# phd3/presto-1

Measured on AMD Instinct MI355X. Metric: probe_rows_per_sec, higher is better.
Workload: dtype int64+f64

## Files before the change

### presto-1_amd/csrc/agg.hip

```cpp
#include "agg.h"
#include "kernels.h"
#include "device_agg.h"

#include <rocprim/rocprim.hpp>

#include <algorithm>
#include <cstdlib>

namespace tgpu {

namespace {

constexpr int kBlock = 256;

struct AggView {
    int32_t function;
    int32_t pad;
    const void *input;
    const uint8_t *input_nulls;
    const uint8_t *mask;
    const uint8_t *mask_nulls;
    const void *input2;
    const uint8_t *input2_nulls;
    long long *counts;
// ... 29 lines not shown
                if (cnt == 0) continue;
                atomicAdd((unsigned long long *)&a.counts[g], (unsigned long long)cnt);
                if (a.function == TGPU_AGG_SUM_BIGINT) i128_add(&a.i128[g * 2], ((const long long *)a.input2)[r]);
                else if (tg_is_minmax(a.function)) tg_minmax_update(&a.i128[g * 2], tg_minmax_encode(a.function, ((const unsigned long long *)a.input2)[r]));
                else kulisch_add(&a.limbs[g * kLimbs], &a.special[g], ((const double *)a.input2)[r]);
                continue;
            }
            if (a.mask && ((a.mask_nulls && a.mask_nulls[r]) || !a.mask[r])) continue;
            if (a.function == TGPU_AGG_COUNT_ALL) {
                atomicAdd((unsigned long long *)&a.counts[g], 1ULL);
                continue;
            }
            if (a.input_nulls && a.input_nulls[r]) continue;
            atomicAdd((unsigned long long *)&a.counts[g], 1ULL);
            switch (a.function) {
            case TGPU_AGG_SUM_BIGINT: i128_add(&a.i128[g * 2], ((const long long *)a.input)[r]); break;
            case TGPU_AGG_MIN_BIGINT:
            case TGPU_AGG_MAX_BIGINT:
            case TGPU_AGG_MIN_DOUBLE:
            case TGPU_AGG_MAX_DOUBLE: tg_minmax_update(&a.i128[g * 2], tg_minmax_encode(a.function, ((const unsigned long long *)a.input)[r])); break;
            case TGPU_AGG_SUM_DOUBLE:
            case TGPU_AGG_AVG_DOUBLE: kulisch_add(&a.limbs[g * kLimbs], &a.special[g], ((const double *)a.input)[r]); break;
            case TGPU_AGG_AVG_BIGINT: kulisch_add(&a.limbs[g * kLimbs], &a.special[g], (double)((const long long *)a.input)[r]); break;
            default: break;
            }
        }
    }
}


__global__ void __launch_bounds__(kBlock) ordered_keys_kernel(const int32_t *__restrict__ gids, int64_t n, unsigned int *__restrict__ keys, int *__restrict__ rows,
                                                               unsigned int *__restrict__ unsorted)
{
    bool bad = false;
    for (int64_t r = (int64_t)blockIdx.x * kBlock + threadIdx.x; r < n; r += (int64_t)gridDim.x * kBlock) {
        const int32_t g = gids[r];
        keys[r] = (unsigned int)(g + 1);
        rows[r] = (int)r;
        bad = bad || (r > 0 && gids[r - 1] > g);
    }
    if (unsorted && __any(bad) && (threadIdx.x & 63) == 0) *unsorted = 1u;
}

__global__ void __launch_bounds__(kBlock) ordered_stretches_kernel(const unsigned int *__restrict__ keys, int64_t n, int *__restrict__ stretches)
{
    for (int64_t i = (int64_t)blockIdx.x * kBlock + threadIdx.x; i < n; i += (int64_t)gridDim.x * kBlock) {
        const unsigned int k = keys[i];
        if (k == 0) continue;
        if (i == 0 || keys[i - 1] != k) stretches[(size_t)(k - 1) * 2] = (int)i;
        if (i == n - 1 || keys[i + 1] != k) stretches[(size_t)(k - 1) * 2 + 1] = (int)(i + 1);
    }
}

template <bool INTERMEDIATE>
__global__ void __launch_bounds__(kBlock) agg_ordered_kernel(AggArgs args, const unsigned int *__restrict__ keys, const int *__restrict__ rows, int64_t n,
                                                              unsigned int *error, int64_t handoff, long long *list, unsigned int *list_count)
{
    for (int64_t i = (int64_t)blockIdx.x * kBlock + threadIdx.x; i < n; i += (int64_t)gridDim.x * kBlock) {
        const unsigned int key = keys[i];
        if (key == 0 || (i > 0 && keys[i - 1] == key)) continue;
        const int64_t g = (int64_t)key - 1;
        const int64_t stop = handoff > 0 ? (i + handoff < n ? i + handoff : n) : n;
        if (handoff > 0 && stop < n && keys[stop] == key) {
            const unsigned int at = atomicAdd(list_count, 1u);
            list[(size_t)at * 2] = g;
            list[(size_t)at * 2 + 1] = stop;
        }
#pragma unroll
        for (int k = 0; k < kMaxAggs; k++) {
            if (k >= args.n_aggs) break;
            const AggView &a = args.a[k];
            long long cnt = 0;
            double s = a.dsum ? a.dsum[g] : 0.0;
            __int128 big = 0;
            unsigned long long best = 0;
            for (int64_t j = i; j < stop && keys[j] == key; j++) {
                const int64_t r = rows[j];
                if (INTERMEDIATE) {
                    const long long c = ((const long long *)a.input)[r];
                    if (c == 0) continue;
                    cnt += c;
                    if (a.function == TGPU_AGG_SUM_BIGINT) big += ((const long long *)a.input2)[r];
                    else if (tg_is_minmax(a.function)) {
                        const unsigned long long c_ = tg_minmax_encode(a.function, ((const unsigned long long *)a.input2)[r]);
                        best = c_ > best ? c_ : best;
                    }
                    else if (a.function != TGPU_AGG_COUNT_ALL && a.function != TGPU_AGG_COUNT_COLUMN) s += ((const double *)a.input2)[r];
                    continue;
                }
                if (a.mask && ((a.mask_nulls && a.mask_nulls[r]) || !a.mask[r])) continue;
                if (a.function != TGPU_AGG_COUNT_ALL && a.input_nulls && a.input_nulls[r]) continue;
                cnt++;
                switch (a.function) {
                case TGPU_AGG_SUM_BIGINT: big += ((const long long *)a.input)[r]; break;
                case TGPU_AGG_MIN_BIGINT:
                case TGPU_AGG_MAX_BIGINT:
                case TGPU_AGG_MIN_DOUBLE:
                case TGPU_AGG_MAX_DOUBLE: {
                    const unsigned long long c_ = tg_minmax_encode(a.function, ((const unsigned long long *)a.input)[r]);
                    best = c_ > best ? c_ : best;
                    break;
                }
                case TGPU_AGG_SUM_DOUBLE:
                case TGPU_AGG_AVG_DOUBLE: s += ((const double *)a.input)[r]; break;
                case TGPU_AGG_AVG_BIGINT: s += (double)((const long long *)a.input)[r]; break;
                default: break;
                }
            }
            if (cnt) a.counts[g] += cnt;
            if (a.dsum) a.dsum[g] = s;
            if (best) tg_minmax_update(&a.i128[g * 2], best);
            if (a.i128 && big != 0) {
                const unsigned __int128 cur = ((unsigned __int128)a.i128[g * 2 + 1] << 64) | a.i128[g * 2];
                const unsigned __int128 nxt = cur + (unsigned __int128)big;
                a.i128[g * 2] = (unsigned long long)nxt;
                a.i128[g * 2 + 1] = (unsigned long long)(nxt >> 64);
            }
        }
    }
    (void)error;
}

struct OrdChainPlan {
    int32_t slot[kMaxAggs];
};

__device__ inline long long wave_sum_i64(long long v)
{
#pragma unroll
    for (int d = 32; d >= 1; d >>= 1) v += __shfl_xor(v, d, 64);
    return v;
}

__device__ inline void ordered_chain_group(const AggArgs &args, const OrdChainPlan &plan, const int *__restrict__ rows, int64_t g, long long s, long long e, double *vals,
                                           unsigned long long *cnt_lds, unsigned long long *lo_lds, long long *hi_lds)
{
    const int wave = threadIdx.x >> 6, lane = threadIdx.x & 63;
    if (threadIdx.x < kMaxAggs) {
        cnt_lds[threadIdx.x] = 0;
        lo_lds[threadIdx.x] = 0;
        hi_lds[threadIdx.x] = 0;
    }
    double *sum = nullptr;
    if (wave == 0) {
        __builtin_amdgcn_s_setprio(3);
#pragma unroll
        for (int k = 0; k < kMaxAggs; k++)
            if (k < args.n_aggs && plan.slot[k] == lane) sum = args.a[k].dsum;
    }
    double os = sum ? sum[g] : 0.0;
    __syncthreads();
    const long long tiles = (e - s + TG_ORD_TILE - 1) / TG_ORD_TILE;
    const int r = (wave - 1) * 64 + lane;
    long long row_next = (wave > 0 && s + r < e) ? rows[s + r] : 0;
    for (long long t = 0; t <= tiles; t++) {
        if (wave > 0 && t < tiles) {
            const long long j = s + t * TG_ORD_TILE + r;
            const long long row = row_next;
            if (j + TG_ORD_TILE < e) row_next = rows[j + TG_ORD_TILE];
            double *out = vals + (t & 1) * (TG_ORD_MAX_DOUBLES * TG_ORD_STRIDE) + r;
            const bool live = j < e;
#pragma unroll
            for (int k = 0; k < kMaxAggs; k++) {
                if (k >= args.n_aggs) break;
                const AggView &a = args.a[k];
                bool take = live;
                if (take && a.mask && ((a.mask_nulls && a.mask_nulls[row]) || !a.mask[row])) take = false;
                if (take && a.function != TGPU_AGG_COUNT_ALL && a.input_nulls && a.input_nulls[row]) take = false;
                const unsigned long long taken = __ballot(take);
                if (lane == 0 && taken) atomicAdd(&cnt_lds[k], (unsigned long long)__popcll(taken));
                if (a.function == TGPU_AGG_SUM_BIGINT) {
                    const long long v = take ? ((const long long *)a.input)[row] : 0;
                    const long long lo = wave_sum_i64((long long)(unsigned int)v), hi = wave_sum_i64(v >> 32);
                    if (lane == 0 && taken) {
                        atomicAdd(&lo_lds[k], (unsigned long long)lo);
                        atomicAdd((unsigned long long *)&hi_lds[k], (unsigned long long)hi);
                    }
                }
                else if (tg_is_minmax(a.function)) {
                    if (take) tg_minmax_update(&a.i128[g * 2], tg_minmax_encode(a.function, ((const unsigned long long *)a.input)[row]));
                }
                else if (plan.slot[k] >= 0 && live) {
                    double x = -0.0;
                    if (take) x = a.function == TGPU_AGG_AVG_BIGINT ? (double)((const long long *)a.input)[row] : ((const double *)a.input)[row];
                    out[plan.slot[k] * TG_ORD_STRIDE] = x;
                }
            }
        }
        else if (wave == 0 && t > 0 && sum) {
            const long long left = e - (s + (t - 1) * TG_ORD_TILE);
            os = tg_chain_add_tile(vals + ((t - 1) & 1) * (TG_ORD_MAX_DOUBLES * TG_ORD_STRIDE) + lane * TG_ORD_STRIDE, left < TG_ORD_TILE ? (int)left : TG_ORD_TILE, os);
        }
        __syncthreads();
    }
    if (sum) sum[g] = os;
    if (threadIdx.x == 64) {
#pragma unroll
        for (int k = 0; k < kMaxAggs; k++) {
            if (k >= args.n_aggs) break;
            const AggView &a = args.a[k];
            if (cnt_lds[k]) a.counts[g] += (long long)cnt_lds[k];
            if (a.function == TGPU_AGG_SUM_BIGINT && a.i128) {
                const __int128 big = (__int128)hi_lds[k] * ((__int128)1 << 32) + (__int128)lo_lds[k];
                const unsigned __int128 cur = ((unsigned __int128)a.i128[g * 2 + 1] << 64) | a.i128[g * 2];
                const unsigned __int128 nxt = cur + (unsigned __int128)big;
                a.i128[g * 2] = (unsigned long long)nxt;
                a.i128[g * 2 + 1] = (unsigned long long)(nxt >> 64);
            }
        }
    }
    __syncthreads();
}

__global__ void __launch_bounds__(TG_ORD_WAVES * 64) agg_ordered_chain_kernel(AggArgs args, OrdChainPlan plan, const int *__restrict__ stretches,
                                                                               const unsigned int *__restrict__ keys, const int *__restrict__ rows, int64_t n,
                                                                               const long long *__restrict__ list, const unsigned int *__restrict__ list_count)
{
    __shared__ __attribute__((aligned(16))) double vals[2 * TG_ORD_MAX_DOUBLES * TG_ORD_STRIDE];
    __shared__ unsigned long long cnt_lds[kMaxAggs], lo_lds[kMaxAggs];
    __shared__ long long hi_lds[kMaxAggs];
    if (stretches) {
        const long long s = stretches[(size_t)blockIdx.x * 2], e = stretches[(size_t)blockIdx.x * 2 + 1];
        if (e > s) ordered_chain_group(args, plan, rows, blockIdx.x, s, e, vals, cnt_lds, lo_lds, hi_lds);
        return;
    }
    const unsigned int count = *list_count;
    for (unsigned int b = blockIdx.x; b < count; b += gridDim.x) {
        const long long g = list[(size_t)b * 2], s = list[(size_t)b * 2 + 1];
        long long lo = s, hi = n;
        while (lo < hi) { const long long mid = (lo + hi) >> 1; if (keys[mid] <= (unsigned int)(g + 1)) lo = mid + 1; else hi = mid; }
        if (lo > s) ordered_chain_group(args, plan, rows, g, s, lo, vals, cnt_lds, lo_lds, hi_lds);
    }
}

using LowCardPlan = TgLowCardPlan;

struct LowCardStates {
    TgAggState st[kMaxAggs];
};

__global__ void __launch_bounds__(kBlock) agg_lowcard_kernel(AggArgs args, LowCardStates states, LowCardPlan plan, const int32_t *__restrict__ gids, int64_t n,
                                                              TgFoldScratch fold)
{
    extern __shared__ __attribute__((aligned(16))) unsigned char lds[];
    tg_lc_zero(lds, plan);
    for (int64_t r = (int64_t)blockIdx.x * kBlock + threadIdx.x; r < n; r += (int64_t)gridDim.x * kBlock) {
        const int g = gids ? gids[r] : 0;
        if (g < 0) continue;
        double *hi_base = tg_lc_hi(lds, plan, g), *lo_base = tg_lc_lo(lds, plan, g);
        unsigned int *cnt_base = tg_lc_cnt(lds, plan, g);
        for (int k = 0; k < args.n_aggs; k++) {
            const AggView &a = args.a[k];
            if (a.mask && ((a.mask_nulls && a.mask_nulls[r]) || !a.mask[r])) continue;
            if (a.function != TGPU_AGG_COUNT_ALL && a.input_nulls && a.input_nulls[r]) continue;
            cnt_base[plan.cnt_slot[k] * kBlock + threadIdx.x] += 1u;
            if (tg_is_minmax(a.function)) {
                tg_minmax_update(&a.i128[(size_t)g * 2], tg_minmax_encode(a.function, ((const unsigned long long *)a.input)[r]));
                continue;
            }
            const int w = plan.wide_slot[k];
            if (w < 0) continue;
            if (a.function == TGPU_AGG_SUM_BIGINT) {
                tg_lc_add_bigint(hi_base, lo_base, w, ((const long long *)a.input)[r]);
                continue;
            }
            const double v = a.function == TGPU_AGG_AVG_BIGINT ? (double)((const long long *)a.input)[r] : ((const double *)a.input)[r];
            if (!(fabs(v) <= 1.7976931348623157e308)) {
                tg_flag_special(&a.special[g], v);
                continue;
            }
            const double r = tg_lc_add_double(hi_base, lo_base, w, v);
            if (r != 0.0) tg_kulisch_add(&a.limbs[(size_t)g * kLimbs], &a.special[g], r);
        }
    }
    tg_lc_fold(lds, plan, states.st, fold);
}

__global__ void __launch_bounds__(kBlock) agg_fold_flush_kernel(TgFoldScratch fs, int rows, int n_aggs, LowCardStates states)
{
    tg_fold_flush(fs, rows, n_aggs, states.st);
}

struct KulischWindow {
    int top;
// ... 517 lines not shown
    HIP_CHECK(rocprim::radix_sort_pairs(temp->ptr(), temp_bytes, keys_in->as<unsigned int>(), keys->as<unsigned int>(), rows_in->as<int>(), rows->as<int>(), (size_t)n, 0,
                                        end_bit, ctx_->stream()));
}

void GroupedAccumulators::add_input(const int32_t *gids, int64_t n, const DevicePage &page, int64_t group_count, bool gids_ascending)
{
    if (states_.empty() || n <= 0) return;
    BufferPtr zero_gids;
    if (!gids && force_ordered()) {
        zero_gids = ctx_->alloc_zero((size_t)n * 4);
        gids = zero_gids->as<int32_t>();
    }
    if (gids) decide_mode(group_count > 0 ? group_count : 1, (160 * 1024) / std::max<int64_t>(lowcard_bytes_per_group(specs()), 1));
    else if (mode_ == Mode::UNDECIDED) mode_ = Mode::EXACT;
    {
        const int64_t lowcard_capacity = (160 * 1024) / std::max<int64_t>(lowcard_bytes_per_group(specs()), 1);
        const int64_t g = group_count > 0 ? group_count : 1;
        ensure(mode_ == Mode::EXACT && g <= lowcard_capacity ? lowcard_capacity : g);
    }
    AggArgs args{};
    args.n_aggs = (int32_t)states_.size();
    for (size_t k = 0; k < states_.size(); k++) {
        State &st = states_[k];
        AggView &a = args.a[k];
        a.function = st.spec.function;
        if (st.spec.function != TGPU_AGG_COUNT_ALL) {
            int32_t want = 0;
            if (bigint_valued(st.spec.function) || st.spec.function == TGPU_AGG_AVG_BIGINT) want = TGPU_BIGINT;
            if (st.spec.function == TGPU_AGG_MIN_DOUBLE || st.spec.function == TGPU_AGG_MAX_DOUBLE) want = TGPU_DOUBLE;
            if (st.spec.function == TGPU_AGG_SUM_DOUBLE || st.spec.function == TGPU_AGG_AVG_DOUBLE) want = TGPU_DOUBLE;
            check_channel(page, st.spec.input_channel, want, "aggregate input");
            a.input = page.cols[st.spec.input_channel].values;
            a.input_nulls = page.cols[st.spec.input_channel].nulls;
        }
        if (st.spec.mask_channel >= 0) {
            check_channel(page, st.spec.mask_channel, TGPU_BOOLEAN, "aggregate mask");
            a.mask = (const uint8_t *)page.cols[st.spec.mask_channel].values;
            a.mask_nulls = page.cols[st.spec.mask_channel].nulls;
        }
        a.counts = st.counts->as<long long>();
        a.limbs = st.limbs ? st.limbs->as<long long>() : nullptr;
        a.special = st.special ? st.special->as<unsigned int>() : nullptr;
        a.i128 = st.i128 ? st.i128->as<unsigned long long>() : nullptr;
        a.dsum = st.dsum ? st.dsum->as<double>() : nullptr;
    }
    if (mode_ == Mode::ORDERED) {
        TG_CHECK_STATE(gids != nullptr, "ordered accumulation needs group ids");
        OrdChainPlan plan{};
        int doubles = 0;
        for (int k = 0; k < kMaxAggs; k++) plan.slot[k] = (k < args.n_aggs && args.a[k].dsum) ? doubles++ : -1;
        const int64_t ids = group_count > 0 ? group_count : 1;
        const bool chained = doubles <= TG_ORD_MAX_DOUBLES && ids <= ord_chain_max_groups() && n >= ids * kOrdChainMinRows && getenv("TGPU_DISABLE_ORDERED_CHAIN") == nullptr;
        ProfileScope ps(ctx_, chained ? "agg_accumulate_ordered_chain" : "agg_accumulate_ordered");
        BufferPtr keys, rows;
        sort_rows_by_group(gids, n, group_count, keys, rows, gids_ascending);
        if (chained) {
            BufferPtr stretches = group_stretches(keys->as<unsigned int>(), n, ids);
            agg_ordered_chain_kernel<<<(int)ids, TG_ORD_WAVES * 64, 0, ctx_->stream()>>>(args, plan, stretches->as<int>(), keys->as<unsigned int>(), rows->as<int>(), n, nullptr,
                                                                                          nullptr);
            check_launch("agg_accumulate_ordered_chain");
            return;
        }
        const int64_t long_groups = n / kOrdHandoffRows;
        const bool handoff = long_groups > 0 && doubles <= TG_ORD_MAX_DOUBLES && getenv("TGPU_DISABLE_ORDERED_CHAIN") == nullptr;
        BufferPtr list = handoff ? ctx_->alloc((size_t)long_groups * 16) : nullptr, list_count = handoff ? ctx_->alloc_zero(8) : nullptr;
        agg_ordered_kernel<false><<<grid_for(ctx_, n), kBlock, 0, ctx_->stream()>>>(args, keys->as<unsigned int>(), rows->as<int>(), n, error_->as<unsigned int>(),
                                                                                      handoff ? kOrdHandoffRows : 0, handoff ? list->as<long long>() : nullptr,
                                                                                      handoff ? list_count->as<unsigned int>() : nullptr);
        check_launch("agg_accumulate_ordered");
        if (handoff) {
            agg_ordered_chain_kernel<<<(int)std::min<int64_t>(long_groups, ctx_->cu_count()), TG_ORD_WAVES * 64, 0, ctx_->stream()>>>(
                args, plan, nullptr, keys->as<unsigned int>(), rows->as<int>(), n, list->as<long long>(), list_count->as<unsigned int>());
            check_launch("agg_accumulate_ordered_handoff");
        }
        return;
    }
    LowCardPlan plan{};
    plan.n_aggs = args.n_aggs;
    for (int k = 0; k < args.n_aggs; k++) {
        plan.wide_slot[k] = (is_count(args.a[k].function) || is_minmax(args.a[k].function)) ? -1 : plan.n_wide++;
        plan.cnt_slot[k] = k;
        plan.count_from_rows[k] = 0;
    }
    plan.n_cnt = plan.n_aggs;
    plan.rows_slot = -1;
    plan.per_group_bytes = plan.n_wide * 2 * kBlock * 8 + plan.n_cnt * kBlock * 4;
    const int64_t groups = group_count > 0 ? group_count : 1;
    const int64_t lds_bytes = groups * plan.per_group_bytes;
    const bool lowcard_enabled = getenv("TGPU_DISABLE_LOWCARD") == nullptr;
    if (lowcard_enabled && lds_bytes <= 160 * 1024 && n >= 4096) {
        plan.n_groups = (int32_t)groups;
        static bool attr_set = false;
        if (!attr_set) {
            HIP_CHECK(hipFuncSetAttribute((const void *)agg_lowcard_kernel, hipFuncAttributeMaxDynamicSharedMemorySize, 160 * 1024));
            attr_set = true;
        }
        const int per_cu = (int)std::max<int64_t>(1, std::min<int64_t>(8, (160 * 1024) / lds_bytes));
        int64_t blocks = std::min<int64_t>((int64_t)ctx_->cu_count() * per_cu, ceil_div(n, kBlock));
        ProfileScope ps(ctx_, "agg_accumulate_lowcard");
        LowCardStates states{};
        for (int k = 0; k < args.n_aggs; k++) {
            states.st[k].function = args.a[k].function;
            states.st[k].counts = args.a[k].counts;
            states.st[k].limbs = args.a[k].limbs;
            states.st[k].special = args.a[k].special;
            states.st[k].i128 = args.a[k].i128;
            states.st[k].dsum = nullptr;
        }
        const FoldScratch fs = fold_scratch(blocks, (160 * 1024) / plan.per_group_bytes);
        agg_lowcard_kernel<<<(int)blocks, kBlock, (size_t)lds_bytes, ctx_->stream()>>>(args, states, plan, gids, n, TgFoldScratch{fs.partials, fs.stride, nullptr});
        check_launch("agg_accumulate_lowcard");
        return;
    }
    ProfileScope ps(ctx_, "agg_accumulate");
    agg_accumulate_kernel<false><<<grid_for(ctx_, n), kBlock, 0, ctx_->stream()>>>(args, gids, n);
    check_launch("agg_accumulate");
}

void GroupedAccumulators::add_intermediate(const int32_t *gids, int64_t n, const DevicePage &page, int64_t group_count, bool gids_ascending)
{
    if (states_.empty() || n <= 0) return;
    BufferPtr zero_gids;
    if (!gids && force_ordered()) {
        zero_gids = ctx_->alloc_zero((size_t)n * 4);
        gids = zero_gids->as<int32_t>();
    }
    if (gids) decide_mode(group_count > 0 ? group_count : 1, (160 * 1024) / std::max<int64_t>(lowcard_bytes_per_group(specs()), 1));
    else if (mode_ == Mode::UNDECIDED) mode_ = Mode::EXACT;
    ensure(group_count > 0 ? group_count : 1);
    AggArgs args{};
    args.n_aggs = (int32_t)states_.size();
    for (size_t k = 0; k < states_.size(); k++) {
        State &st = states_[k];
        AggView &a = args.a[k];
        a.function = st.spec.function;
        int ch = st.spec.input_channel;
        check_channel(page, ch, TGPU_BIGINT, "intermediate count");
        a.input = page.cols[ch].values;
        ch++;
        if (!is_count(st.spec.function)) {
            check_channel(page, ch, bigint_valued(st.spec.function) ? TGPU_BIGINT : TGPU_DOUBLE, "intermediate sum");
            a.input2 = page.cols[ch].values;
            ch++;
        }
        a.counts = st.counts->as<long long>();
        a.limbs = st.limbs ? st.limbs->as<long long>() : nullptr;
        a.special = st.special ? st.special->as<unsigned int>() : nullptr;
        a.i128 = st.i128 ? st.i128->as<unsigned long long>() : nullptr;
        a.dsum = st.dsum ? st.dsum->as<double>() : nullptr;
    }
    if (mode_ == Mode::ORDERED) {
        TG_CHECK_STATE(gids != nullptr, "ordered accumulation needs group ids");
        ProfileScope ps(ctx_, "agg_combine_ordered");
        BufferPtr keys, rows;
        sort_rows_by_group(gids, n, group_count, keys, rows, gids_ascending && zero_gids == nullptr);
        agg_ordered_kernel<true><<<grid_for(ctx_, n), kBlock, 0, ctx_->stream()>>>(args, keys->as<unsigned int>(), rows->as<int>(), n, error_->as<unsigned int>(), 0, nullptr,
                                                                                     nullptr);
        check_launch("agg_combine_ordered");
        return;
    }
    ProfileScope ps(ctx_, "agg_combine");
    agg_accumulate_kernel<true><<<grid_for(ctx_, n), kBlock, 0, ctx_->stream()>>>(args, gids, n);
    check_launch("agg_combine");
}

void GroupedAccumulators::evaluate(int64_t groups, std::vector<DeviceColumn> &out)
{
    if (states_.empty()) return;
    ensure(groups > 0 ? groups : 1);
    flush_fold();
    EvalArgs args{};
    args.n_aggs = (int32_t)states_.size();
    const bool partial = step_ == TGPU_STEP_PARTIAL;
    const int64_t alloc_n = groups > 0 ? groups : 1;
    for (size_t k = 0; k < states_.size(); k++) {
        State &st = states_[k];
        EvalView &a = args.a[k];
        a.function = st.spec.function;
        a.partial = partial ? 1 : 0;
        a.counts = st.counts->as<long long>();
        a.limbs = st.limbs ? st.limbs->as<long long>() : nullptr;
        a.special = st.special ? st.special->as<unsigned int>() : nullptr;
        a.i128 = st.i128 ? st.i128->as<unsigned long long>() : nullptr;
        a.dsum = st.dsum ? st.dsum->as<double>() : nullptr;
        DeviceColumn c0;
        c0.n = groups;
        c0.values_buf = ctx_->alloc((size_t)alloc_n * 8);
        c0.values = c0.values_buf->ptr();
        a.out0 = c0.values_buf->ptr();
        if (is_count(st.spec.function) || partial) {
            c0.type = TGPU_BIGINT;
            out.push_back(c0);
            if (partial && !is_count(st.spec.function)) {
                DeviceColumn c1;
                c1.n = groups;
                c1.type = bigint_valued(st.spec.function) ? TGPU_BIGINT : TGPU_DOUBLE;
                c1.values_buf = ctx_->alloc((size_t)alloc_n * 8);
                c1.values = c1.values_buf->ptr();
                a.out1 = c1.values_buf->ptr();
                out.push_back(c1);
            }
        }
        else {
            c0.type = bigint_valued(st.spec.function) ? TGPU_BIGINT : TGPU_DOUBLE;
            c0.nulls_buf = ctx_->alloc((size_t)alloc_n);
            c0.nulls = c0.nulls_buf->as<uint8_t>();
            a.out0_nulls = c0.nulls_buf->as<uint8_t>();
            out.push_back(c0);
        }
    }
// ... 17 lines not shown
```

### presto-1_amd/csrc/basic.hip

```cpp
#include "kernels.h"
#include "device_hash.h"

namespace tgpu {
namespace k {

constexpr int kBlock = 256;
constexpr int kWaves = kBlock / 64;

constexpr int kScanItems = 8;
constexpr int kScanTile = kBlock * kScanItems;

template <typename T> __device__ __forceinline__ T wave_inclusive_scan(T v)
{
    const int lane = threadIdx.x & 63;
#pragma unroll
    for (int d = 1; d < 64; d <<= 1) {
        T t = __shfl_up(v, d, 64);
        if (lane >= d) v += t;
    }
    return v;
}

template <typename T> __device__ __forceinline__ T block_exclusive_scan(T v, T *total, T *lds )
{
// ... 43 lines not shown
    block_exclusive_scan<int64_t>(s, &total, lds);
    if (threadIdx.x == 0) range_sums[blockIdx.x] = total;
}

__global__ void __launch_bounds__(kBlock) scan_ranges_i32(const int32_t *__restrict__ in, int32_t *__restrict__ out, int64_t n, int64_t range,
                                                           const int64_t *__restrict__ range_prefix)
{
    __shared__ int64_t lds[kWaves + 1];
    const bool aligned = (reinterpret_cast<uintptr_t>(in) & 15) == 0, out_aligned = (reinterpret_cast<uintptr_t>(out) & 15) == 0;
    const int64_t a = (int64_t)blockIdx.x * range, z = a + range < n ? a + range : n;
    int64_t carry = range_prefix[blockIdx.x];
    for (int64_t base = a; base < z; base += kScanTile) {
        const int64_t idx = base + (int64_t)threadIdx.x * kScanItems;
        int32_t v[kScanItems];
        scan_load8(in, idx, z, aligned, v);
        int64_t s = 0;
#pragma unroll
        for (int i = 0; i < kScanItems; i++) s += v[i];
        int64_t total;
        int64_t prefix = carry + block_exclusive_scan<int64_t>(s, &total, lds);
        int32_t o[kScanItems];
#pragma unroll
        for (int i = 0; i < kScanItems; i++) {
            o[i] = (int32_t)prefix;
            prefix += v[i];
        }
        if (out_aligned && idx + kScanItems <= z) {
            *reinterpret_cast<int4 *>(out + idx) = make_int4(o[0], o[1], o[2], o[3]);
            *reinterpret_cast<int4 *>(out + idx + 4) = make_int4(o[4], o[5], o[6], o[7]);
        } else {
#pragma unroll
            for (int i = 0; i < kScanItems; i++)
                if (idx + i < z) out[idx + i] = o[i];
        }
        carry += total;
    }
}

__global__ void __launch_bounds__(kBlock) scan_small_i64(const int64_t *__restrict__ in, int64_t *__restrict__ out, int64_t n, int64_t *total_out)
{
    __shared__ int64_t lds[kWaves + 1];
    int64_t carry = 0;
    for (int64_t base = 0; base < n; base += kBlock) {
        int64_t idx = base + threadIdx.x;
        int64_t v = idx < n ? in[idx] : 0;
        int64_t total;
        int64_t p = block_exclusive_scan<int64_t>(v, &total, lds);
        if (idx < n) out[idx] = carry + p;
        carry += total;
    }
    if (threadIdx.x == 0 && total_out) *total_out = carry;
}

__global__ void __launch_bounds__(kBlock) scan_one_tile_i32(const int32_t *__restrict__ in, int32_t *__restrict__ out, int64_t n, int64_t *total_out)
{
    __shared__ int64_t lds[kWaves + 1];
    const int64_t base = (int64_t)threadIdx.x * kScanItems;
    int32_t v[kScanItems];
    int64_t s = 0;
#pragma unroll
    for (int i = 0; i < kScanItems; i++) {
        v[i] = base + i < n ? in[base + i] : 0;
        s += v[i];
    }
    int64_t total;
    int64_t prefix = block_exclusive_scan<int64_t>(s, &total, lds);
#pragma unroll
    for (int i = 0; i < kScanItems; i++) {
        if (base + i < n) out[base + i] = (int32_t)prefix;
        prefix += v[i];
    }
    if (threadIdx.x == 0 && total_out) *total_out = total;
}

void exclusive_scan_i32(Context *ctx, const int32_t *in, int32_t *out, int64_t n, int64_t *total_dev)
{
    if (n <= 0) {
        if (total_dev) HIP_CHECK(hipMemsetAsync(total_dev, 0, 8, ctx->stream()));
        return;
    }
    if (n <= kScanTile) {
        scan_one_tile_i32<<<1, kBlock, 0, ctx->stream()>>>(in, out, n, total_dev);
        check_launch("exclusive_scan_i32");
        return;
    }
    const int64_t tiles = ceil_div(n, kScanTile);
    const int64_t tiles_per_range = ceil_div(tiles, (int64_t)kScanMaxBlocks), range = tiles_per_range * kScanTile, ranges = ceil_div(n, range);
    BufferPtr sums = ctx->alloc((size_t)ranges * 8);
    BufferPtr prefix = ctx->alloc((size_t)ranges * 8);
    scan_range_sums_i32<<<(int)ranges, kBlock, 0, ctx->stream()>>>(in, n, range, sums->as<int64_t>());
    scan_small_i64<<<1, kBlock, 0, ctx->stream()>>>(sums->as<int64_t>(), prefix->as<int64_t>(), ranges, total_dev);
    scan_ranges_i32<<<(int)ranges, kBlock, 0, ctx->stream()>>>(in, out, n, range, prefix->as<int64_t>());
    check_launch("exclusive_scan_i32");
}

__global__ void __launch_bounds__(kBlock) hash_rows_kernel(KeyCols keys, int64_t n, int64_t *__restrict__ out)
{
    for (int64_t r = (int64_t)blockIdx.x * kBlock + threadIdx.x; r < n; r += (int64_t)gridDim.x * kBlock) {
        out[r] = tg_hash_row_u(keys, r);
    }
}

void hash_rows(Context *ctx, const KeyCols &keys, int64_t n, int64_t *out)
{
    if (n <= 0) return;
    ProfileScope ps(ctx, "hash_rows");
    hash_rows_kernel<<<grid_for(ctx, n), kBlock, 0, ctx->stream()>>>(keys, n, out);
    check_launch("hash_rows");
}

__global__ void __launch_bounds__(kBlock) any_null_kernel(KeyCols keys, int64_t n, uint8_t *__restrict__ out)
{
    for (int64_t r = (int64_t)blockIdx.x * kBlock + threadIdx.x; r < n; r += (int64_t)gridDim.x * kBlock) {
        uint8_t f = 0;
#pragma unroll
        for (int c = 0; c < TG_MAX_KEY_CHANNELS; c++) {
            if (c >= keys.n) break;
            f |= (keys.c[c].nulls && keys.c[c].nulls[r]) ? 1 : 0;
        }
        out[r] = f;
    }
}

void any_null(Context *ctx, const KeyCols &keys, int64_t n, uint8_t *out)
{
    if (n <= 0) return;
    any_null_kernel<<<grid_for(ctx, n), kBlock, 0, ctx->stream()>>>(keys, n, out);
    check_launch("any_null");
}

template <typename T> __global__ void __launch_bounds__(kBlock) fill_kernel(T *p, T v, int64_t n)
{
    for (int64_t i = (int64_t)blockIdx.x * kBlock + threadIdx.x; i < n; i += (int64_t)gridDim.x * kBlock) p[i] = v;
}
__global__ void __launch_bounds__(kBlock) iota_kernel(int32_t *p, int64_t n)
// ... 188 lines not shown
```

### presto-1_amd/csrc/join.hip

```cpp
#include "join.h"
#include "kernels.h"
#include "device_hash.h"
#include "device_join.h"

#include <rocprim/rocprim.hpp>

#include <algorithm>
#include <cstdlib>

namespace tgpu {

namespace {

constexpr int kBlock = 256;

using Slot16 = TgSlot16;

__device__ __forceinline__ bool rows_equal_nonnull(const KeyCols &a, int64_t ra, const KeyCols &b, int64_t rb)
{
#pragma unroll
    for (int c = 0; c < TG_MAX_KEY_CHANNELS; c++) {
        if (c >= a.n) break;
        const ColView &x = a.c[c], &y = b.c[c];
        switch (x.type) {
// ... 299 lines not shown
            const long long up = __shfl_up(k[u], 1, 64);
            const long long pred = lane == 0 ? before[u] : up;
            descent = descent || (r < n && r > 0 && pred >= k[u]);
        }
    }
    block_minmax(lo, hi, minmax);
    if (__any(descent) && (threadIdx.x & 63) == 0) minmax[2] = 1;
}

__global__ void __launch_bounds__(kBlock) build_direct_kernel(ColView key, int64_t n, long long key_min, unsigned long long *bitmap,
                                                               unsigned long long *counters)
{
    const int lane = threadIdx.x & 63;
    unsigned int my_dups = 0;
    for (int64_t base = (int64_t)blockIdx.x * kBlock; base < n; base += (int64_t)gridDim.x * kBlock) {
        const int64_t r = base + threadIdx.x;
        const bool active = r < n && !(key.nulls && key.nulls[r]);
        unsigned long long d = 0;
        if (active) {
            d = (unsigned long long)int_key_at(key, r) - (unsigned long long)key_min;
        }
        const unsigned int word = active ? (unsigned int)(d >> 6) : 0xffffffffu;
        unsigned long long bits = active ? (1ULL << (d & 63)) : 0ULL;
        unsigned int rows = active ? 1u : 0u;
        const unsigned int word_prev = __shfl_up(word, 1, 64);
        const bool head = lane == 0 || word_prev != word;
        const unsigned long long heads = __ballot(head);
        const int run = __popcll(heads & ((2ULL << lane) - 1ULL));
#pragma unroll
        for (int k = 1; k < 64; k <<= 1) {
            const unsigned long long b2 = __shfl_down(bits, k, 64);
            const unsigned int c2 = __shfl_down(rows, k, 64);
            const int run2 = __shfl_down(run, k, 64);
            if (lane + k < 64 && run2 == run) {
                bits |= b2;
                rows += c2;
            }
        }
        if (head && active) {
            const unsigned long long old = atomicOr(&bitmap[word], bits);
            my_dups += (unsigned int)__popcll(old & bits) + (rows - (unsigned int)__popcll(bits));
        }
    }
    __shared__ unsigned int s_dups[kBlock / 64];
#pragma unroll
    for (int d = 32; d >= 1; d >>= 1) my_dups += __shfl_down(my_dups, d, 64);
    if (lane == 0) s_dups[threadIdx.x >> 6] = my_dups;
    __syncthreads();
    if (threadIdx.x == 0) {
        unsigned long long total = 0;
#pragma unroll
        for (int w = 0; w < kBlock / 64; w++) total += s_dups[w];
        if (total) atomicAdd(&counters[0], total);
    }
}

__global__ void __launch_bounds__(kBlock) init_slots_kernel(Slot16 *__restrict__ slots, int64_t capacity)
{
    for (int64_t i = (int64_t)blockIdx.x * kBlock + threadIdx.x; i < capacity; i += (int64_t)gridDim.x * kBlock) {
        Slot16 s;
        s.key = kUnwrittenKey;
        s.head = -1;
        s.count = 1;
        slots[i] = s;
    }
}

__global__ void __launch_bounds__(kBlock) bitmap_popcount_kernel(const unsigned long long *__restrict__ bitmap, int64_t words, int32_t *__restrict__ counts)
{
    for (int64_t i = (int64_t)blockIdx.x * kBlock + threadIdx.x; i < words; i += (int64_t)gridDim.x * kBlock) counts[i] = (int32_t)__popcll(bitmap[i]);
}

__global__ void __launch_bounds__(kBlock) build_rank_kernel(ColView key, int64_t n, long long key_min, const unsigned long long *__restrict__ bitmap,
                                                             const int32_t *__restrict__ rank_base, int32_t *__restrict__ direct)
{
    for (int64_t r = (int64_t)blockIdx.x * kBlock + threadIdx.x; r < n; r += (int64_t)gridDim.x * kBlock) {
        if (key.nulls && key.nulls[r]) continue;
        const unsigned long long d = (unsigned long long)int_key_at(key, r) - (unsigned long long)key_min;
        direct[rank_base[d >> 6] + __popcll(bitmap[d >> 6] & ((1ULL << (d & 63)) - 1ULL))] = (int32_t)r;
    }
}

__global__ void __launch_bounds__(kBlock) bitmap_build_kernel(const int32_t *__restrict__ row_slot, int64_t n, ColView key, long long key_min,
                                                               unsigned long long *bitmap)
{
    for (int64_t r = (int64_t)blockIdx.x * kBlock + threadIdx.x; r < n; r += (int64_t)gridDim.x * kBlock) {
        if (row_slot[r] < 0) continue;
        const unsigned long long d = (unsigned long long)(int_key_at(key, r) - key_min);
        atomicOr(&bitmap[d >> 6], 1ULL << (d & 63));
    }
}

__global__ void __launch_bounds__(kBlock) bloom_build_kernel(const int32_t *__restrict__ row_slot, int64_t n, ColView key, unsigned long long *bloom,
                                                              unsigned long long word_mask)
{
    for (int64_t r = (int64_t)blockIdx.x * kBlock + threadIdx.x; r < n; r += (int64_t)gridDim.x * kBlock) {
        if (row_slot[r] < 0) continue;
        const unsigned long long m = tg_fmix64((unsigned long long)tg_hash_long(int_key_at(key, r)));
        atomicOr(&bloom[tg_bloom_word(m, word_mask)], tg_bloom_mask(m));
    }
}

struct ProbeTable {
    const int *heads;
    const Slot16 *slots;
    const uint8_t *tags;
// ... 359 lines not shown
        links_kernel<<<g, kBlock, 0, ctx_->stream()>>>(keys_out->as<unsigned long long>(), n_, links_->as<int32_t>(), int_key_fast_ ? slots16_->as<Slot16>() : nullptr);
        check_launch("links");
    }
    if (int_key_fast_) {
        ProfileScope ps(ctx_, "join_build_prefilter");
        key_min_ = (long long)host_ctr[2];
        key_max_ = (long long)host_ctr[3];
        const bool has_keys = key_max_ >= key_min_;
        const unsigned long long range = has_keys ? (unsigned long long)key_max_ - (unsigned long long)key_min_ + 1ULL : 0ULL;
        const bool dense = has_keys && range != 0 && range <= (1ULL << 34) && range / 4096ULL <= (unsigned long long)std::max<int64_t>(n_, 1) &&
                           getenv("TGPU_DISABLE_BITMAP") == nullptr;
        if (dense) {
            const int64_t words = (int64_t)((range + 63) / 64);
            bitmap_ = ctx_->alloc_zero((size_t)words * 8);
            bitmap_build_kernel<<<g, kBlock, 0, ctx_->stream()>>>(row_slot->as<int32_t>(), n_, keys.c[0], key_min_, bitmap_->as<unsigned long long>());
            check_launch("bitmap_build");
        }
        else if (has_keys) {
            static const int bits_per_key = getenv("TGPU_BLOOM_BITS_PER_KEY") ? std::max(1, atoi(getenv("TGPU_BLOOM_BITS_PER_KEY"))) : 16;
            int64_t words = 1024;
            while (words * 64 < n_ * bits_per_key) words <<= 1;
            static const int64_t max_bloom_bytes = getenv("TGPU_BLOOM_MAX_BYTES") ? atoll(getenv("TGPU_BLOOM_MAX_BYTES")) : (1ll << 40);
            if (words * 8 <= max_bloom_bytes) {
                bloom_words_ = words;
                bloom_ = ctx_->alloc_zero((size_t)words * 8);
                bloom_build_kernel<<<g, kBlock, 0, ctx_->stream()>>>(row_slot->as<int32_t>(), n_, keys.c[0], bloom_->as<unsigned long long>(), (unsigned long long)words - 1);
                check_launch("bloom_build");
            }
        }
    }
}

bool LookupSourceGpu::build_direct(const KeyCols &keys)
{
    const int g = grid_for(ctx_, n_);
    BufferPtr mm = ctx_->alloc(24);
    const long long init[3] = {0x7fffffffffffffffLL, -0x7fffffffffffffffLL - 1, 0};
    ctx_->upload(mm->ptr(), init, 24);
    long long host_mm[3];
    {
        ProfileScope ps(ctx_, "join_build_range");
        key_range_kernel<<<std::min(g, ctx_->cu_count() * 2), kBlock, 0, ctx_->stream()>>>(keys.c[0], n_, mm->as<long long>());
        check_launch("key_range");
    }
    ctx_->download(host_mm, mm->ptr(), 24);
    if (host_mm[1] < host_mm[0]) return false;
    const bool ascending = host_mm[2] == 0 && keys.c[0].nulls == nullptr && getenv("TGPU_DISABLE_ASCENDING_BUILD") == nullptr;
    const unsigned long long range = (unsigned long long)host_mm[1] - (unsigned long long)host_mm[0] + 1ULL;
    if (range == 0 || range > (1ULL << 31) || range / 64ULL > (unsigned long long)n_) return false;
    const int64_t words = (int64_t)((range + 63) / 64);
    BufferPtr bitmap = ctx_->alloc_zero((size_t)words * 8);
    BufferPtr direct = ascending ? nullptr : ctx_->alloc((size_t)n_ * 4);
    BufferPtr rank_base = ctx_->alloc((size_t)words * 4);
    BufferPtr counters = ctx_->alloc_zero(16);
    {
        ProfileScope ps(ctx_, "join_build_insert");
        build_direct_kernel<<<g, kBlock, 0, ctx_->stream()>>>(keys.c[0], n_, host_mm[0], bitmap->as<unsigned long long>(), counters->as<unsigned long long>());
        check_launch("build_direct");
    }
    if (!ascending && ctx_->read_scalar(counters->as<unsigned long long>()) != 0) return false;
    key_min_ = host_mm[0];
    key_max_ = host_mm[1];
    bitmap_ = bitmap;
    direct_ = direct;
    rank_base_ = rank_base;
    direct_key_ = keys.c[0];
    rank_pending_ = true;
    if (!output_channels_.empty()) ensure_rank();
    return true;
}

void LookupSourceGpu::ensure_rank() const
{
    if (!rank_base_) return;
    std::lock_guard<std::mutex> lk(visited_mu_);
    if (!rank_pending_) return;
    const int64_t range = (int64_t)((unsigned long long)key_max_ - (unsigned long long)key_min_ + 1ULL);
    const int64_t words = (range + 63) / 64;
    ProfileScope ps(ctx_, "join_build_rank");
    BufferPtr counts = ctx_->alloc((size_t)words * 4), total = ctx_->alloc(8);
    bitmap_popcount_kernel<<<grid_for(ctx_, words), kBlock, 0, ctx_->stream()>>>(bitmap_->as<unsigned long long>(), words, counts->as<int32_t>());
    check_launch("bitmap_popcount");
    k::exclusive_scan_i32(ctx_, counts->as<int32_t>(), rank_base_->as<int32_t>(), words, total->as<int64_t>());
    if (direct_) {
        build_rank_kernel<<<grid_for(ctx_, n_), kBlock, 0, ctx_->stream()>>>(direct_key_, n_, key_min_, bitmap_->as<unsigned long long>(), rank_base_->as<int32_t>(),
                                                                            direct_->as<int32_t>());
        check_launch("build_rank");
    }
    rank_pending_ = false;
}

bool LookupSourceGpu::int_table(IntTableView &v) const
{
    if (!int_key_fast_ || (!slots16_ && !rank_base_)) return false;
    v.slots = slots16_ ? slots16_->ptr() : nullptr;
    v.direct = direct_ ? direct_->as<int32_t>() : nullptr;
    v.rank_base = rank_base_ ? rank_base_->as<int32_t>() : nullptr;
    v.mask = (uint64_t)capacity_ - 1;
    v.bloom = bloom_ ? bloom_->as<unsigned long long>() : nullptr;
    v.bloom_word_mask = bloom_ ? (unsigned long long)bloom_words_ - 1 : 0;
    v.bitmap = bitmap_ ? bitmap_->as<unsigned long long>() : nullptr;
    v.key_min = key_min_;
    v.key_max = key_max_;
    v.links = links_ ? links_->as<int32_t>() : nullptr;
    v.key_type = key_cols_.empty() ? index_->types()[(size_t)key_channels_[0]] : key_cols_[0].type;
    return true;
}

void LookupSourceGpu::probe(const std::vector<const DeviceColumn *> &probe_keys, const int64_t *probe_hashes, int64_t n, bool probe_outer,
                            BufferPtr &out_probe_idx, BufferPtr &out_build_idx, int64_t &out_count)
{
    TG_CHECK_ARG(probe_keys.size() == key_channels_.size(), "probe key channel count differs from the build side's");
    for (size_t i = 0; i < probe_keys.size(); i++) {
        const int32_t bt = index_->types()[key_channels_[i]];
        const bool int_like = (bt == TGPU_BIGINT || bt == TGPU_INTEGER || bt == TGPU_DATE);
        TG_CHECK_ARG(probe_keys[i]->type == bt || (int_key_fast_ && int_like && probe_keys[i]->type == bt), "probe key type differs from the build key type");
    }
    out_count = 0;
    if (n <= 0) {
        out_probe_idx = ctx_->alloc(4);
        out_build_idx = ctx_->alloc(4);
// ... 120 lines not shown
```

Measured before the change: 86.10 billion.

## Skip group sort for ascending ids, fuse direct-build rank, loop single-block scan

When group ids are already ascending, ordered aggregation now walks the id array directly through a templated accessor, with row index equal to position, so the sort_rows_by_group pass is skipped. The direct-join build for ascending keys now uses a wave-level kernel that merges bits per bitmap word, issues one atomic OR per word, and writes the word's first row as rank_base, so the separate popcount and scan rank pass is dropped. The single-block i32 scan now loops over tiles with prefetching and vector stores, and covers inputs up to a larger bound to avoid the multi-block path. The risks are that correctness depends on the ascending flags being accurate, and that one block is now serial over larger scans.

```diff
diff --git a/presto-1_amd/csrc/agg.hip b/presto-1_amd/csrc/agg.hip
--- a/presto-1_amd/csrc/agg.hip
+++ b/presto-1_amd/csrc/agg.hip
@@ -105,16 +105,28 @@
     }
 }
 
-template <bool INTERMEDIATE>
-__global__ void __launch_bounds__(kBlock) agg_ordered_kernel(AggArgs args, const unsigned int *__restrict__ keys, const int *__restrict__ rows, int64_t n,
-                                                              unsigned int *error, int64_t handoff, long long *list, unsigned int *list_count)
+struct OrdPairs {
+    const unsigned int *__restrict__ keys;
+    const int *__restrict__ rows;
+    __device__ __forceinline__ unsigned int key(int64_t j) const { return keys[j]; }
+    __device__ __forceinline__ int64_t row(int64_t j) const { return rows[j]; }
+};
+struct OrdIds {
+    const int32_t *__restrict__ gids;
+    __device__ __forceinline__ unsigned int key(int64_t j) const { return (unsigned int)(gids[j] + 1); }
+    __device__ __forceinline__ int64_t row(int64_t j) const { return j; }
+};
+
+template <bool INTERMEDIATE, typename ORD>
+__global__ void __launch_bounds__(kBlock) agg_ordered_kernel(AggArgs args, ORD ord, int64_t n, unsigned int *error, int64_t handoff, long long *list,
+                                                              unsigned int *list_count)
 {
     for (int64_t i = (int64_t)blockIdx.x * kBlock + threadIdx.x; i < n; i += (int64_t)gridDim.x * kBlock) {
-        const unsigned int key = keys[i];
-        if (key == 0 || (i > 0 && keys[i - 1] == key)) continue;
+        const unsigned int key = ord.key(i);
+        if (key == 0 || (i > 0 && ord.key(i - 1) == key)) continue;
         const int64_t g = (int64_t)key - 1;
         const int64_t stop = handoff > 0 ? (i + handoff < n ? i + handoff : n) : n;
-        if (handoff > 0 && stop < n && keys[stop] == key) {
+        if (handoff > 0 && stop < n && ord.key(stop) == key) {
             const unsigned int at = atomicAdd(list_count, 1u);
             list[(size_t)at * 2] = g;
             list[(size_t)at * 2 + 1] = stop;
@@ -127,8 +139,8 @@
             double s = a.dsum ? a.dsum[g] : 0.0;
             __int128 big = 0;
             unsigned long long best = 0;
-            for (int64_t j = i; j < stop && keys[j] == key; j++) {
-                const int64_t r = rows[j];
+            for (int64_t j = i; j < stop && ord.key(j) == key; j++) {
+                const int64_t r = ord.row(j);
                 if (INTERMEDIATE) {
                     const long long c = ((const long long *)a.input)[r];
                     if (c == 0) continue;
@@ -185,7 +197,8 @@
     return v;
 }
 
-__device__ inline void ordered_chain_group(const AggArgs &args, const OrdChainPlan &plan, const int *__restrict__ rows, int64_t g, long long s, long long e, double *vals,
+template <typename ORD>
+__device__ inline void ordered_chain_group(const AggArgs &args, const OrdChainPlan &plan, const ORD &ord, int64_t g, long long s, long long e, double *vals,
                                            unsigned long long *cnt_lds, unsigned long long *lo_lds, long long *hi_lds)
 {
     const int wave = threadIdx.x >> 6, lane = threadIdx.x & 63;
@@ -205,12 +218,12 @@
     __syncthreads();
     const long long tiles = (e - s + TG_ORD_TILE - 1) / TG_ORD_TILE;
     const int r = (wave - 1) * 64 + lane;
-    long long row_next = (wave > 0 && s + r < e) ? rows[s + r] : 0;
+    long long row_next = (wave > 0 && s + r < e) ? ord.row(s + r) : 0;
     for (long long t = 0; t <= tiles; t++) {
         if (wave > 0 && t < tiles) {
             const long long j = s + t * TG_ORD_TILE + r;
             const long long row = row_next;
-            if (j + TG_ORD_TILE < e) row_next = rows[j + TG_ORD_TILE];
+            if (j + TG_ORD_TILE < e) row_next = ord.row(j + TG_ORD_TILE);
             double *out = vals + (t & 1) * (TG_ORD_MAX_DOUBLES * TG_ORD_STRIDE) + r;
             const bool live = j < e;
 #pragma unroll
@@ -265,8 +278,8 @@
     __syncthreads();
 }
 
-__global__ void __launch_bounds__(TG_ORD_WAVES * 64) agg_ordered_chain_kernel(AggArgs args, OrdChainPlan plan, const int *__restrict__ stretches,
-                                                                               const unsigned int *__restrict__ keys, const int *__restrict__ rows, int64_t n,
+template <typename ORD>
+__global__ void __launch_bounds__(TG_ORD_WAVES * 64) agg_ordered_chain_kernel(AggArgs args, OrdChainPlan plan, const int *__restrict__ stretches, ORD ord, int64_t n,
                                                                                const long long *__restrict__ list, const unsigned int *__restrict__ list_count)
 {
     __shared__ __attribute__((aligned(16))) double vals[2 * TG_ORD_MAX_DOUBLES * TG_ORD_STRIDE];
@@ -274,15 +287,15 @@
     __shared__ long long hi_lds[kMaxAggs];
     if (stretches) {
         const long long s = stretches[(size_t)blockIdx.x * 2], e = stretches[(size_t)blockIdx.x * 2 + 1];
-        if (e > s) ordered_chain_group(args, plan, rows, blockIdx.x, s, e, vals, cnt_lds, lo_lds, hi_lds);
+        if (e > s) ordered_chain_group(args, plan, ord, blockIdx.x, s, e, vals, cnt_lds, lo_lds, hi_lds);
         return;
     }
     const unsigned int count = *list_count;
     for (unsigned int b = blockIdx.x; b < count; b += gridDim.x) {
         const long long g = list[(size_t)b * 2], s = list[(size_t)b * 2 + 1];
         long long lo = s, hi = n;
-        while (lo < hi) { const long long mid = (lo + hi) >> 1; if (keys[mid] <= (unsigned int)(g + 1)) lo = mid + 1; else hi = mid; }
-        if (lo > s) ordered_chain_group(args, plan, rows, g, s, lo, vals, cnt_lds, lo_lds, hi_lds);
+        while (lo < hi) { const long long mid = (lo + hi) >> 1; if (ord.key(mid) <= (unsigned int)(g + 1)) lo = mid + 1; else hi = mid; }
+        if (lo > s) ordered_chain_group(args, plan, ord, g, s, lo, vals, cnt_lds, lo_lds, hi_lds);
     }
 }
 
@@ -906,27 +919,32 @@
         const int64_t ids = group_count > 0 ? group_count : 1;
         const bool chained = doubles <= TG_ORD_MAX_DOUBLES && ids <= ord_chain_max_groups() && n >= ids * kOrdChainMinRows && getenv("TGPU_DISABLE_ORDERED_CHAIN") == nullptr;
         ProfileScope ps(ctx_, chained ? "agg_accumulate_ordered_chain" : "agg_accumulate_ordered");
+        const bool from_ids = gids_ascending && !chained && getenv("TGPU_ALWAYS_SORT") == nullptr;
         BufferPtr keys, rows;
-        sort_rows_by_group(gids, n, group_count, keys, rows, gids_ascending);
+        if (!from_ids) sort_rows_by_group(gids, n, group_count, keys, rows, gids_ascending);
         if (chained) {
             BufferPtr stretches = group_stretches(keys->as<unsigned int>(), n, ids);
-            agg_ordered_chain_kernel<<<(int)ids, TG_ORD_WAVES * 64, 0, ctx_->stream()>>>(args, plan, stretches->as<int>(), keys->as<unsigned int>(), rows->as<int>(), n, nullptr,
-                                                                                          nullptr);
+            agg_ordered_chain_kernel<<<(int)ids, TG_ORD_WAVES * 64, 0, ctx_->stream()>>>(args, plan, stretches->as<int>(), OrdPairs{keys->as<unsigned int>(), rows->as<int>()}, n,
+                                                                                          nullptr, nullptr);
             check_launch("agg_accumulate_ordered_chain");
             return;
         }
         const int64_t long_groups = n / kOrdHandoffRows;
         const bool handoff = long_groups > 0 && doubles <= TG_ORD_MAX_DOUBLES && getenv("TGPU_DISABLE_ORDERED_CHAIN") == nullptr;
         BufferPtr list = handoff ? ctx_->alloc((size_t)long_groups * 16) : nullptr, list_count = handoff ? ctx_->alloc_zero(8) : nullptr;
-        agg_ordered_kernel<false><<<grid_for(ctx_, n), kBlock, 0, ctx_->stream()>>>(args, keys->as<unsigned int>(), rows->as<int>(), n, error_->as<unsigned int>(),
-                                                                                      handoff ? kOrdHandoffRows : 0, handoff ? list->as<long long>() : nullptr,
-                                                                                      handoff ? list_count->as<unsigned int>() : nullptr);
-        check_launch("agg_accumulate_ordered");
-        if (handoff) {
-            agg_ordered_chain_kernel<<<(int)std::min<int64_t>(long_groups, ctx_->cu_count()), TG_ORD_WAVES * 64, 0, ctx_->stream()>>>(
-                args, plan, nullptr, keys->as<unsigned int>(), rows->as<int>(), n, list->as<long long>(), list_count->as<unsigned int>());
-            check_launch("agg_accumulate_ordered_handoff");
-        }
+        auto walk = [&](auto ord) {
+            agg_ordered_kernel<false><<<grid_for(ctx_, n), kBlock, 0, ctx_->stream()>>>(args, ord, n, error_->as<unsigned int>(), handoff ? kOrdHandoffRows : 0,
+                                                                                          handoff ? list->as<long long>() : nullptr,
+                                                                                          handoff ? list_count->as<unsigned int>() : nullptr);
+            check_launch("agg_accumulate_ordered");
+            if (handoff) {
+                agg_ordered_chain_kernel<<<(int)std::min<int64_t>(long_groups, ctx_->cu_count()), TG_ORD_WAVES * 64, 0, ctx_->stream()>>>(
+                    args, plan, nullptr, ord, n, list->as<long long>(), list_count->as<unsigned int>());
+                check_launch("agg_accumulate_ordered_handoff");
+            }
+        };
+        if (from_ids) walk(OrdIds{gids});
+        else walk(OrdPairs{keys->as<unsigned int>(), rows->as<int>()});
         return;
     }
     LowCardPlan plan{};
@@ -1006,10 +1024,15 @@
     if (mode_ == Mode::ORDERED) {
         TG_CHECK_STATE(gids != nullptr, "ordered accumulation needs group ids");
         ProfileScope ps(ctx_, "agg_combine_ordered");
+        if (gids_ascending && zero_gids == nullptr && getenv("TGPU_ALWAYS_SORT") == nullptr) {
+            agg_ordered_kernel<true><<<grid_for(ctx_, n), kBlock, 0, ctx_->stream()>>>(args, OrdIds{gids}, n, error_->as<unsigned int>(), 0, nullptr, nullptr);
+            check_launch("agg_combine_ordered");
+            return;
+        }
         BufferPtr keys, rows;
-        sort_rows_by_group(gids, n, group_count, keys, rows, gids_ascending && zero_gids == nullptr);
-        agg_ordered_kernel<true><<<grid_for(ctx_, n), kBlock, 0, ctx_->stream()>>>(args, keys->as<unsigned int>(), rows->as<int>(), n, error_->as<unsigned int>(), 0, nullptr,
-                                                                                     nullptr);
+        sort_rows_by_group(gids, n, group_count, keys, rows);
+        agg_ordered_kernel<true><<<grid_for(ctx_, n), kBlock, 0, ctx_->stream()>>>(args, OrdPairs{keys->as<unsigned int>(), rows->as<int>()}, n, error_->as<unsigned int>(), 0,
+                                                                                     nullptr, nullptr);
         check_launch("agg_combine_ordered");
         return;
     }
diff --git a/presto-1_amd/csrc/basic.hip b/presto-1_amd/csrc/basic.hip
--- a/presto-1_amd/csrc/basic.hip
+++ b/presto-1_amd/csrc/basic.hip
@@ -119,25 +119,48 @@
     if (threadIdx.x == 0 && total_out) *total_out = carry;
 }
 
-__global__ void __launch_bounds__(kBlock) scan_one_tile_i32(const int32_t *__restrict__ in, int32_t *__restrict__ out, int64_t n, int64_t *total_out)
+__global__ void __launch_bounds__(kBlock) scan_one_block_i32(const int32_t *__restrict__ in, int32_t *__restrict__ out, int64_t n, int64_t *total_out)
 {
     __shared__ int64_t lds[kWaves + 1];
-    const int64_t base = (int64_t)threadIdx.x * kScanItems;
-    int32_t v[kScanItems];
-    int64_t s = 0;
-#pragma unroll
-    for (int i = 0; i < kScanItems; i++) {
-        v[i] = base + i < n ? in[base + i] : 0;
-        s += v[i];
-    }
-    int64_t total;
-    int64_t prefix = block_exclusive_scan<int64_t>(s, &total, lds);
-#pragma unroll
-    for (int i = 0; i < kScanItems; i++) {
-        if (base + i < n) out[base + i] = (int32_t)prefix;
-        prefix += v[i];
-    }
-    if (threadIdx.x == 0 && total_out) *total_out = total;
+    const bool aligned = (reinterpret_cast<uintptr_t>(in) & 15) == 0, out_aligned = (reinterpret_cast<uintptr_t>(out) & 15) == 0;
+    int64_t carry = 0;
+    int32_t v[kScanItems], next[kScanItems];
+    scan_load8(in, (int64_t)threadIdx.x * kScanItems, n, aligned, next);
+    for (int64_t base = 0; base < n; base += kScanTile) {
+        const int64_t idx = base + (int64_t)threadIdx.x * kScanItems;
+#pragma unroll
+        for (int i = 0; i < kScanItems; i++) v[i] = next[i];
+        if (base + kScanTile < n) scan_load8(in, idx + kScanTile, n, aligned, next);
+        int64_t s = 0;
+#pragma unroll
+        for (int i = 0; i < kScanItems; i++) s += v[i];
+        int64_t total;
+        int64_t prefix = carry + block_exclusive_scan<int64_t>(s, &total, lds);
+        int32_t o[kScanItems];
+#pragma unroll
+        for (int i = 0; i < kScanItems; i++) {
+            o[i] = (int32_t)prefix;
+            prefix += v[i];
+        }
+        if (out_aligned && idx + kScanItems <= n) {
+            *reinterpret_cast<int4 *>(out + idx) = make_int4(o[0], o[1], o[2], o[3]);
+            *reinterpret_cast<int4 *>(out + idx + 4) = make_int4(o[4], o[5], o[6], o[7]);
+        } else {
+#pragma unroll
+            for (int i = 0; i < kScanItems; i++)
+                if (idx + i < n) out[idx + i] = o[i];
+        }
+        carry += total;
+    }
+    if (threadIdx.x == 0 && total_out) *total_out = carry;
+}
+
+constexpr int64_t kScanOneBlockMax = 16384;
+
+static int64_t scan_one_block_max()
+{
+    const char *e = getenv("TGPU_SCAN_ONE_BLOCK_MAX");
+    return std::max<int64_t>(e ? atoll(e) : kScanOneBlockMax, kScanTile);
 }
 
 void exclusive_scan_i32(Context *ctx, const int32_t *in, int32_t *out, int64_t n, int64_t *total_dev)
@@ -146,8 +169,8 @@
         if (total_dev) HIP_CHECK(hipMemsetAsync(total_dev, 0, 8, ctx->stream()));
         return;
     }
-    if (n <= kScanTile) {
-        scan_one_tile_i32<<<1, kBlock, 0, ctx->stream()>>>(in, out, n, total_dev);
+    if (n <= scan_one_block_max()) {
+        scan_one_block_i32<<<1, kBlock, 0, ctx->stream()>>>(in, out, n, total_dev);
         check_launch("exclusive_scan_i32");
         return;
     }
diff --git a/presto-1_amd/csrc/join.hip b/presto-1_amd/csrc/join.hip
--- a/presto-1_amd/csrc/join.hip
+++ b/presto-1_amd/csrc/join.hip
@@ -375,6 +375,36 @@
 #pragma unroll
         for (int w = 0; w < kBlock / 64; w++) total += s_dups[w];
         if (total) atomicAdd(&counters[0], total);
+    }
+}
+
+template <bool RANK>
+__global__ void __launch_bounds__(kBlock) build_direct_ascending_kernel(ColView key, int64_t n, long long key_min, unsigned long long *bitmap,
+                                                                         int32_t *__restrict__ rank_base)
+{
+    const int lane = threadIdx.x & 63;
+    for (int64_t base = (int64_t)blockIdx.x * kBlock; base < n; base += (int64_t)gridDim.x * kBlock) {
+        const int64_t r = base + threadIdx.x;
+        const bool active = r < n;
+        const unsigned long long d = active ? (unsigned long long)int_key_at(key, r) - (unsigned long long)key_min : 0ULL;
+        const unsigned int before = (lane == 0 && active && r > 0) ? (unsigned int)(((unsigned long long)int_key_at(key, r - 1) - (unsigned long long)key_min) >> 6) : 0xffffffffu;
+        const unsigned int word = active ? (unsigned int)(d >> 6) : 0xffffffffu;
+        unsigned long long bits = active ? (1ULL << (d & 63)) : 0ULL;
+        const unsigned int up = __shfl_up(word, 1, 64);
+        const bool first = (lane == 0 ? before : up) != word;
+        const bool head = lane == 0 || first;
+        const unsigned long long heads = __ballot(head);
+        const int run = __popcll(heads & ((2ULL << lane) - 1ULL));
+#pragma unroll
+        for (int k = 1; k < 64; k <<= 1) {
+            const unsigned long long b2 = __shfl_down(bits, k, 64);
+            const int run2 = __shfl_down(run, k, 64);
+            if (lane + k < 64 && run2 == run) bits |= b2;
+        }
+        if (head && active) {
+            __hip_atomic_fetch_or(&bitmap[word], bits, __ATOMIC_RELAXED, __HIP_MEMORY_SCOPE_AGENT);
+            if (RANK && first) rank_base[word] = (int32_t)r;
+        }
     }
 }
 
@@ -840,10 +870,17 @@
     BufferPtr bitmap = ctx_->alloc_zero((size_t)words * 8);
     BufferPtr direct = ascending ? nullptr : ctx_->alloc((size_t)n_ * 4);
     BufferPtr rank_base = ctx_->alloc((size_t)words * 4);
-    BufferPtr counters = ctx_->alloc_zero(16);
+    const bool one_pass = ascending && getenv("TGPU_DIRECT_RANK_SCAN") == nullptr;
+    const bool want_rank = !output_channels_.empty();
+    BufferPtr counters = one_pass ? nullptr : ctx_->alloc_zero(16);
     {
         ProfileScope ps(ctx_, "join_build_insert");
-        build_direct_kernel<<<g, kBlock, 0, ctx_->stream()>>>(keys.c[0], n_, host_mm[0], bitmap->as<unsigned long long>(), counters->as<unsigned long long>());
+        if (one_pass && want_rank)
+            build_direct_ascending_kernel<true><<<g, kBlock, 0, ctx_->stream()>>>(keys.c[0], n_, host_mm[0], bitmap->as<unsigned long long>(), rank_base->as<int32_t>());
+        else if (one_pass)
+            build_direct_ascending_kernel<false><<<g, kBlock, 0, ctx_->stream()>>>(keys.c[0], n_, host_mm[0], bitmap->as<unsigned long long>(), nullptr);
+        else
+            build_direct_kernel<<<g, kBlock, 0, ctx_->stream()>>>(keys.c[0], n_, host_mm[0], bitmap->as<unsigned long long>(), counters->as<unsigned long long>());
         check_launch("build_direct");
     }
     if (!ascending && ctx_->read_scalar(counters->as<unsigned long long>()) != 0) return false;
@@ -853,8 +890,8 @@
     direct_ = direct;
     rank_base_ = rank_base;
     direct_key_ = keys.c[0];
-    rank_pending_ = true;
-    if (!output_channels_.empty()) ensure_rank();
+    rank_pending_ = !(one_pass && want_rank);
+    if (want_rank) ensure_rank();
     return true;
 }
 
```

Measured after the change: 88.22 billion, median of 6. 1.02x the previous value.
